# bioscan-ml/bioscan-clip

Hardware: AMD Instinct MI355X
Metric: paired samples/sec/node (I+D+T, global batch) + step MFMA-roofline % at 1/2/4/8 GPU (higher is better)
Workload: dtype bf16; 1 GPU; configs[2]: Image+DNA+Text (LoRA ViT-B/16 + LoRA BarcodeBERT + BERT-small), local batch 256, 224x224 images + 133-token barcodes, local-batch InfoNCE, fused AdamW; local_batch=256, global_batch=256, parallelism=dp1, collectives=none (one process, local-batch loss)

## Files before the change

### bioscan-clip_amd/csrc/common.h

```cpp
#pragma once
#include <hip/hip_runtime.h>
#include <stdint.h>

#include "../../include/bsclip.h"

typedef unsigned short bf16_t;
typedef __attribute__((ext_vector_type(8))) __bf16 bf16x8;
typedef __attribute__((ext_vector_type(4))) float f32x4;
typedef __attribute__((ext_vector_type(16))) float f32x16;
typedef __attribute__((ext_vector_type(4))) unsigned short u16x4;
typedef __attribute__((ext_vector_type(8))) unsigned short u16x8;

#define BSCLIP_WAVE 64

void bsclip_set_error(const char* fmt, ...);
#define BSCLIP_REQUIRE(cond, ...)                    \
    do {                                             \
        if (!(cond)) {                               \
            bsclip_set_error(__VA_ARGS__);           \
            return BSCLIP_ERR_INVALID;               \
        }                                            \
    } while (0)
#define BSCLIP_LAUNCH_CHECK()                                                        \
    do {                                                                             \
// ... 217 lines not shown
}

static inline int ceil_div(int a, int b) { return (a + b - 1) / b; }

void bsclip_launch_slab_reduce_add(const float* partial, int nblocks, int n, float* out0, float* out1, int split, hipStream_t s);

void bsclip_launch_attn_fwd_x3(const float* qkv, int ld_qkv, int B, int S, int heads, const float* key_bias, float scale, float* ctx,
                               int ld_ctx, float* lse, const DropCfg& drop, bf16_t* ctx3, int ld_c3, hipStream_t s);
void bsclip_launch_attn_bwd_x3(const float* qkv, int ld_qkv, const float* dctx, int ld_dctx, const float* ctx, int ld_ctx, const float* lse,
                               int B, int S, int heads, const float* key_bias, float scale, float* dqkv, int ld_dqkv, const DropCfg& drop,
                               bf16_t* dqkv3, int ld_d3, hipStream_t s);

int bsclip_gemm_infonce(int mode, const void* A, int lda, const void* B, int ldb, void* C, int ldc, int M, int N, int K,
                        const int64_t* labels, const float* cnt, const float* lse_row, const float* lse_col, float* part,
                        float logit_scale, float coef, int n_valid, int row_base, void* stream);
```

### bioscan-clip_amd/csrc/gemm.hip

```cpp
#include <type_traits>

#include "common.h"

namespace {

constexpr int BK = 64;
constexpr int ROW_BYTES = BK * 2;

__device__ __forceinline__ int xcd_remap(int orig, int nwg) {
    const int q = nwg >> 3, r = nwg & 7, xcd = orig & 7;
    return (xcd < r ? xcd * (q + 1) : r * (q + 1) + (xcd - r) * q) + (orig >> 3);
}

struct EpiArgs {
    const float* bias;
    const float* resid;
    int ld_resid;
    unsigned char* aux;
    int ld_aux;
    DropCfg drop;
    int n_total;
    unsigned long long* diag;
    int pers_gw;
    const float* alpha;
// ... 131 lines not shown
        v += bf4_to_f32<F16>(r);
        *reinterpret_cast<uint2*>(static_cast<bf16_t*>(C) + (size_t)m * ldc + n) = f32_to_bf4<F16>(v);
    } else if constexpr (EPI == BSCLIP_EPI_PATCH_BF16) {
        const int b = m / 196, p = m - b * 196;
        const f32x4 pos = *reinterpret_cast<const f32x4*>(e.resid + (size_t)(1 + p) * e.ld_resid + n);
        v += pos;
        *reinterpret_cast<uint2*>(static_cast<bf16_t*>(C) + (size_t)(b * 197 + 1 + p) * ldc + n) = f32_to_bf4<F16>(v);
    }
}

template <int BM, int BN, int WAVES_M, int WAVES_N, int EPI, bool HAS_BIAS, bool F16 = false>
__global__ __launch_bounds__(WAVES_M* WAVES_N * 64) void gemm_nt_kernel(const bf16_t* __restrict__ A, int lda,
                                                                         const bf16_t* __restrict__ B, int ldb,
                                                                         void* __restrict__ C, int ldc, int M, int N,
                                                                         int K, int tiles_n, EpiArgs e) {
    constexpr int NW = WAVES_M * WAVES_N;
    constexpr int WTM = BM / WAVES_M, WTN = BN / WAVES_N;
    if constexpr (epi_is_resid(EPI)) BSCLIP_DROP_RESOLVE(e.drop);
    constexpr int TM = WTM / 16, TN = WTN / 16;
    constexpr int A_BYTES = BM * ROW_BYTES, B_BYTES = BN * ROW_BYTES;
    constexpr int STAGE_BYTES = A_BYTES + B_BYTES;
    constexpr int A_PER_WAVE = BM / 8 / NW, B_PER_WAVE = BN / 8 / NW;
    static_assert(BM % (8 * NW) == 0 && BN % (8 * NW) == 0, "staging split");
    __shared__ __attribute__((aligned(16))) char smem[2 * STAGE_BYTES];

    const int wg = xcd_remap(blockIdx.x, gridDim.x);
    const int tile_n = wg % tiles_n, tile_m = wg / tiles_n;
    const int m0 = tile_m * BM, n0 = tile_n * BN;

    const int tid = threadIdx.x, lane = tid & 63;
    const int wave = __builtin_amdgcn_readfirstlane(tid >> 6);
    const int wm = wave / WAVES_N, wn = wave % WAVES_N;

    const bf16_t* a_src[A_PER_WAVE];
    const bf16_t* b_src[B_PER_WAVE];
#pragma unroll
    for (int i = 0; i < A_PER_WAVE; ++i) {
        const int row = (wave + i * NW) * 8 + (lane >> 3);
        const int c = (lane & 7) ^ ((row >> 1) & 7);
        const int grow = min(m0 + row, M - 1);
        a_src[i] = A + (size_t)grow * lda + c * 8;
    }
#pragma unroll
    for (int i = 0; i < B_PER_WAVE; ++i) {
        const int row = (wave + i * NW) * 8 + (lane >> 3);
        const int c = (lane & 7) ^ ((row >> 1) & 7);
        const int grow = min(n0 + row, N - 1);
        b_src[i] = B + (size_t)grow * ldb + c * 8;
    }
    auto stage = [&](int buf, int k0) {
        char* sA = smem + buf * STAGE_BYTES;
        char* sB = sA + A_BYTES;
#pragma unroll
        for (int i = 0; i < A_PER_WAVE; ++i) glds16(a_src[i] + k0, sA + (wave + i * NW) * 1024);
#pragma unroll
        for (int i = 0; i < B_PER_WAVE; ++i) glds16(b_src[i] + k0, sB + (wave + i * NW) * 1024);
    };

    const int fr = lane & 15, fq = lane >> 4;
    const int sw = fr >> 1;
    const int a_off0 = (wm * WTM + fr) * ROW_BYTES + ((fq ^ sw) << 4);
    const int b_off0 = (wn * WTN + fr) * ROW_BYTES + ((fq ^ sw) << 4);

    f32x4 acc[TM][TN];
#pragma unroll
    for (int i = 0; i < TM; ++i)
#pragma unroll
        for (int j = 0; j < TN; ++j) acc[i][j] = f32x4{0.f, 0.f, 0.f, 0.f};

    const int nk = K / BK;
    stage(0, 0);
    __syncthreads();

    for (int t = 0; t < nk; ++t) {
        const int cur = t & 1;
        if (t + 1 < nk) stage(cur ^ 1, (t + 1) * BK);
        const char* sA = smem + cur * STAGE_BYTES;
        const char* sB = sA + A_BYTES;
#pragma unroll
        for (int ks = 0; ks < 2; ++ks) {
            bf16x8 af[TM], bfr[TN];
#pragma unroll
            for (int j = 0; j < TN; ++j)
                bfr[j] = *reinterpret_cast<const bf16x8*>(sB + ((b_off0 ^ (ks << 6)) + j * 16 * ROW_BYTES));
#pragma unroll
            for (int i = 0; i < TM; ++i)
                af[i] = *reinterpret_cast<const bf16x8*>(sA + ((a_off0 ^ (ks << 6)) + i * 16 * ROW_BYTES));
#pragma unroll
            for (int i = 0; i < TM; ++i)
#pragma unroll
                for (int j = 0; j < TN; ++j)
                    acc[i][j] = mfma16x16x32<F16>(bfr[j], af[i], acc[i][j]);
        }
        __syncthreads();
    }

    f32x4 bias[TN];
#pragma unroll
    for (int j = 0; j < TN; ++j) {
        bias[j] = f32x4{0.f, 0.f, 0.f, 0.f};
        if constexpr (HAS_BIAS) bias[j] = *reinterpret_cast<const f32x4*>(e.bias + n0 + wn * WTN + j * 16 + fq * 4);
    }
    if constexpr (HAS_BIAS) {
#pragma unroll
        for (int i = 0; i < TM; ++i)
#pragma unroll
            for (int j = 0; j < TN; ++j) acc[i][j] += bias[j];
    }
    auto store_rows = [&](auto guard) {
#pragma unroll
        for (int i = 0; i < TM; ++i) {
            const int m = m0 + wm * WTM + i * 16 + fr;
            if (!decltype(guard)::value || m < M) {
#pragma unroll
                for (int j = 0; j < TN; ++j) {
                    const int n = n0 + wn * WTN + j * 16 + fq * 4;
                    epilogue_store<EPI, F16>(acc[i][j], m, n, C, ldc, e);
                }
            }
        }
    };
    if (m0 + BM <= M) store_rows(std::false_type{});
    else store_rows(std::true_type{});
}

template <int EPI, bool HAS_BIAS, bool DIAG = false, int ABL = 0, int SCHED = 0, int OP = 0>
__global__ __launch_bounds__(512) void gemm_nt_pp_kernel(const bf16_t* __restrict__ A, int lda,
                                                          const bf16_t* __restrict__ B, int ldb, void* __restrict__ C,
                                                          int ldc, int M, int N, int K, int tiles_n, EpiArgs e) {
    static_assert(OP == 0 || (SCHED == 0 && ABL == 0), "fp8 / fp16 operands: production schedule only");
    constexpr bool FP8 = OP == 1 || OP == 2, F16 = OP == 3;
    if constexpr (EPI == BSCLIP_EPI_F32 && !HAS_BIAS && OP == 0) {
        A += (size_t)blockIdx.y * K;
        B += (size_t)blockIdx.y * K;
        C = static_cast<float*>(C) + (size_t)blockIdx.y * e.split_stride;
    }
    if constexpr (epi_is_resid(EPI)) BSCLIP_DROP_RESOLVE(e.drop);
    constexpr int ESZ = FP8 ? 1 : 2;
// ... 702 lines not shown
    const int tiles_m = ceil_div(M, BM), tiles_n = N / BN;
    hipLaunchKernelGGL((gemm_nt_kernel<BM, BN, WM, WN, EPI, HB, F16>), dim3(tiles_m * tiles_n), dim3(WM * WN * 64), 0, s, A,
                       lda, B, ldb, C, ldc, M, N, K, tiles_n, e);
}

bool g_lut_ready = false;

template <int EPI, bool HB, bool F16, int SCHED = 0>
void launch_pp(const bf16_t* A, int lda, const bf16_t* B, int ldb, void* C, int ldc, int M, int N, int K,
               const EpiArgs& e, hipStream_t s) {
    const int tiles_m = ceil_div(M, 256), tiles_n = N / 256;
    hipLaunchKernelGGL((gemm_nt_pp_kernel<EPI, HB, false, 0, F16 ? 0 : SCHED, F16 ? 3 : 0>), dim3(tiles_m * tiles_n), dim3(512), 0, s, A, lda, B,
                       ldb, C, ldc, M, N, K, tiles_n, e);
}

template <int EPI, bool HB, bool F16>
void launch_epi(const bf16_t* A, int lda, const bf16_t* B, int ldb, void* C, int ldc, int M, int N, int K,
                const EpiArgs& e, hipStream_t s) {
    if (EPI == BSCLIP_EPI_GELU_BF16 && !g_lut_ready) {
        hipLaunchKernelGGL(gelu_lut_init_kernel, dim3(ceil_div(GELU_LUT_N + 1, 256)), dim3(256), 0, s);
        g_lut_ready = true;
    }
    int tile = g_tile_override;
    if (tile == 0) {
        const long t256 = (long)ceil_div(M, 256) * (N / 256);
        if (N % 256 == 0 && t256 >= 192) tile = 4;
        else tile = 1;
        if (tile == 4 && N == 768 && K == 768 && t256 >= 500 && EPI != BSCLIP_EPI_GELU_BF16 && !g_duo_off) tile = 5;
        if (tile == 4 && pers_supported(EPI) && K <= g_pers_max_k && K >= 2 * BK && t256 >= g_pers_min_tiles && !g_pers_off) tile = 8;
    }
    if (F16 && tile == 5) tile = 4;
    if ((tile == 3 || tile == 4 || tile == 6 || tile == 7 || tile == 8) && N % 256 != 0) tile = 2;
    switch (tile) {
        case 4: launch_pp<EPI, HB, F16>(A, lda, B, ldb, C, ldc, M, N, K, e, s); break;
        case 5:
            if constexpr (!F16) launch_duo<EPI, HB>(A, lda, B, ldb, C, ldc, M, N, K, e, s);
            break;
        case 8:
            if constexpr (pers_supported(EPI)) {
                if (K >= 2 * BK && (size_t)M * lda * 2 < (1ull << 32) && (size_t)N * ldb * 2 < (1ull << 32)) {
                    launch_pers<EPI, HB, F16>(A, lda, B, ldb, C, ldc, M, N, K, e, s);
                    break;
                }
            }
            launch_pp<EPI, HB, F16>(A, lda, B, ldb, C, ldc, M, N, K, e, s);
            break;
#ifdef BSCLIP_DIAG
// ... 304 lines not shown
    e.n_total = N;
    e.drop = make_drop(0.f, 0);
    const int tiles_m = ceil_div(M, 256), tiles_n = N / 256;
    hipStream_t s = static_cast<hipStream_t>(stream);
    const bf16_t* a = static_cast<const bf16_t*>(A);
    const bf16_t* b = static_cast<const bf16_t*>(B);
    if (mode == 0) {
        BSCLIP_REQUIRE(part, "bsclip_gemm_infonce: part is null");
        hipLaunchKernelGGL((gemm_nt_pp_kernel<EPI_LSE_PART, false>), dim3(tiles_m * tiles_n), dim3(512), 0, s, a, lda, b, ldb, C,
                           ldc, M, N, K, tiles_n, e);
    } else {
        BSCLIP_REQUIRE(C && cnt && lse_row && lse_col && ldc % 3 == 0, "bsclip_gemm_infonce: pass 2 operands");
        hipLaunchKernelGGL((gemm_nt_pp_kernel<EPI_LOSS_W, false>), dim3(tiles_m * tiles_n), dim3(512), 0, s, a, lda, b, ldb, C,
                           ldc, M, N, K, tiles_n, e);
    }
    BSCLIP_LAUNCH_CHECK();
    return BSCLIP_OK;
}

extern "C" int bsclip_gemm_fp8(const void* A8, int lda, const void* B8, int ldb, void* C, int ldc, int M, int N, int K,
                               int epilogue, const bsclip_epi_args* args, const bsclip_fp8_args* f8, void* stream) {
    BSCLIP_REQUIRE(A8 && B8 && C && args && f8, "bsclip_gemm_fp8: null pointer");
    BSCLIP_REQUIRE(args->struct_size == sizeof(bsclip_epi_args) && f8->struct_size == sizeof(bsclip_fp8_args),
                   "bsclip_gemm_fp8: struct_size mismatch (epi %u/%zu, fp8 %u/%zu)", args->struct_size,
                   sizeof(bsclip_epi_args), f8->struct_size, sizeof(bsclip_fp8_args));
    BSCLIP_REQUIRE(M > 0 && N > 0 && K > 0 && K % 128 == 0 && N % 256 == 0, "bsclip_gemm_fp8: M=%d N=%d K=%d (K %% 128, N %% 256)",
                   M, N, K);
    BSCLIP_REQUIRE(lda >= K && ldb >= K && lda % 16 == 0 && ldb % 16 == 0, "bsclip_gemm_fp8: lda=%d ldb=%d (K=%d)", lda, ldb, K);
    BSCLIP_REQUIRE(ldc >= N && ldc % 4 == 0 && (epilogue != BSCLIP_EPI_GELU_FP8 || ldc % 16 == 0), "bsclip_gemm_fp8: ldc=%d", ldc);
    BSCLIP_REQUIRE((((uintptr_t)A8 | (uintptr_t)B8 | (uintptr_t)C) & 15) == 0, "bsclip_gemm_fp8: 16-B alignment");
// ... 96 lines not shown
```

### bioscan-clip_amd/csrc/loss.hip

```cpp
#include <math.h>

#include "common.h"

namespace {

typedef __attribute__((ext_vector_type(4))) unsigned u32x4;

__device__ __forceinline__ void split_bf(float x, bf16_t& hi, bf16_t& lo) {
    hi = f2bf(x);
    lo = f2bf(x - bf2f(hi));
}

__global__ __launch_bounds__(256) void loss_prep_kernel(const float* __restrict__ z, int N, int Np, int D,
                                                         float* __restrict__ zn, float* __restrict__ inv,
                                                         bf16_t* __restrict__ PA, bf16_t* __restrict__ PB) {
    const int lane = threadIdx.x & 63;
    const int row = (blockIdx.x * 256 + threadIdx.x) >> 6;
    if (row >= Np) return;
    float scale = 0.f;
    if (row < N) {
        float ss = 0.f;
        for (int c = lane * 4; c < D; c += 256) {
            const f32x4 v = *reinterpret_cast<const f32x4*>(z + (size_t)row * D + c);
            ss += (v[0] * v[0] + v[1] * v[1]) + (v[2] * v[2] + v[3] * v[3]);
        }
        ss = wave_sum(ss);
        scale = 1.0f / fmaxf(sqrtf(ss), 1e-12f);
    }
    if (lane == 0) inv[row] = scale;
    for (int c = lane * 4; c < D; c += 256) {
// ... 3 lines not shown
        bf16_t h[4], l[4];
#pragma unroll
        for (int i = 0; i < 4; ++i) split_bf(v[i], h[i], l[i]);
        const uint2 hh = {(unsigned)h[0] | ((unsigned)h[1] << 16), (unsigned)h[2] | ((unsigned)h[3] << 16)};
        const uint2 ll = {(unsigned)l[0] | ((unsigned)l[1] << 16), (unsigned)l[2] | ((unsigned)l[3] << 16)};
        bf16_t* pa = PA + (size_t)row * 3 * D + c;
        bf16_t* pb = PB + (size_t)row * 3 * D + c;
        *reinterpret_cast<uint2*>(pa) = hh;
        *reinterpret_cast<uint2*>(pa + D) = hh;
        *reinterpret_cast<uint2*>(pa + 2 * D) = ll;
        *reinterpret_cast<uint2*>(pb) = hh;
        *reinterpret_cast<uint2*>(pb + D) = ll;
        *reinterpret_cast<uint2*>(pb + 2 * D) = hh;
    }
}

__global__ __launch_bounds__(256) void loss_transpose_split_kernel(const float* __restrict__ zn, int Np, int D,
                                                                    bf16_t* __restrict__ PBt) {
    __shared__ float tile[64][65];
    const int r0 = blockIdx.y * 64, c0 = blockIdx.x * 64;
    const int tx = threadIdx.x & 63, ty = threadIdx.x >> 6;
    for (int i = ty; i < 64; i += 4) tile[i][tx] = zn[(size_t)(r0 + i) * D + c0 + tx];
    __syncthreads();
    for (int i = ty; i < 64; i += 4) {
        const float v = tile[tx][i];
        bf16_t h, l;
        split_bf(v, h, l);
        bf16_t* dst = PBt + (size_t)(c0 + i) * 3 * Np + r0 + tx;
        dst[0] = h;
        dst[Np] = l;
        dst[2 * Np] = h;
    }
}

__global__ void loss_count_kernel(const int64_t* __restrict__ labels, int N, float* __restrict__ cnt) {
    const int i = blockIdx.x * blockDim.x + threadIdx.x;
    if (i >= N) return;
    const int64_t li = labels[i];
    int c = 0;
    for (int j = 0; j < N; ++j) c += (labels[j] == li);
    cnt[i] = (float)c;
}

__global__ __launch_bounds__(256) void loss_row_reduce_kernel(const float* __restrict__ G, int row0, int nrows, int N,
                                                               int Np, float s, const int64_t* __restrict__ labels,
                                                               const float* __restrict__ cnt, float* __restrict__ lse,
                                                               float* __restrict__ contrib) {
    const int lane = threadIdx.x & 63;
    const int r = (blockIdx.x * 256 + threadIdx.x) >> 6;
    if (r >= nrows) return;
    const int row = row0 + r;
    const float* g = G + (size_t)r * Np;
    const int64_t li = labels[row];
    float m = -INFINITY;
    for (int j = lane; j < N; j += 64) m = fmaxf(m, g[j]);
    m = wave_max(m) * s;
    float se = 0.f, dot = 0.f;
    for (int j = lane; j < N; j += 64) {
        const float x = g[j] * s;
        se += __expf(x - m);
        if (labels[j] == li) dot += x;
    }
    se = wave_sum(se);
    dot = wave_sum(dot);
    const float l = m + __logf(se);
    if (lane == 0) {
        lse[row] = l;
        contrib[row] = cnt[row] * l - dot;
    }
}

__global__ __launch_bounds__(256) void loss_w_kernel(const float* __restrict__ G, int N, int Np, int row0, int n_local,
                                                      float s, float coef, const int64_t* __restrict__ labels,
                                                      const float* __restrict__ cnt, const float* __restrict__ lse_ab,
                                                      const float* __restrict__ lse_ba, bf16_t* __restrict__ W) {
    const long total = (long)n_local * Np;
    for (long it = (long)blockIdx.x * 256 + threadIdx.x; it < total; it += (long)gridDim.x * 256) {
        const int il = (int)(it / Np), j = (int)(it % Np);
        float w = 0.f;
        if (j < N) {
            const int i = row0 + il;
            const float x = G[(size_t)il * Np + j] * s;
            const float t = (labels[i] == labels[j]) ? 2.0f : 0.0f;
            w = coef * (cnt[i] * __expf(x - lse_ab[i]) + cnt[j] * __expf(x - lse_ba[j]) - t);
        }
        bf16_t h, l;
        split_bf(w, h, l);
        bf16_t* dst = W + (size_t)il * 3 * Np + j;
        dst[0] = h;
        dst[Np] = h;
        dst[2 * Np] = l;
    }
}

__global__ __launch_bounds__(256) void loss_final_kernel(const float* __restrict__ contrib, int nmod, int Np, int N, float scale,
                                                          float* __restrict__ loss_out) {
    __shared__ float red[256];
    float s = 0.f;
    for (int slot = 0; slot < nmod * nmod; ++slot) {
        if (slot / nmod == slot % nmod) continue;
        for (int i = threadIdx.x; i < N; i += 256) s += contrib[(size_t)slot * Np + i];
    }
    red[threadIdx.x] = s;
    __syncthreads();
    for (int o = 128; o > 0; o >>= 1) {
        if (threadIdx.x < o) red[threadIdx.x] += red[threadIdx.x + o];
        __syncthreads();
// ... 9 lines not shown
    const f32x4* p = reinterpret_cast<const f32x4*>(part) + (size_t)i * tiles;
    float m = -INFINITY;
    for (int t = 0; t < tiles; ++t) m = fmaxf(m, p[t][0]);
    float s = 0.f, dot = 0.f;
    for (int t = 0; t < tiles; ++t) {
        const f32x4 v = p[t];
        s += v[0] == -INFINITY ? 0.f : v[1] * __expf(v[0] - m);
        dot += v[2];
    }
    const float l = m + __logf(s);
    lse[i] = l;
    contrib[i] = cnt[i] * l - dot;
}

int g_infonce_impl = 0;

inline int64_t align4(int64_t x) { return (x + 3) & ~(int64_t)3; }

constexpr int SLAB_ROWS = 1024;

struct Layout {
    int Np, slab;
    int64_t zn, inv, PA, PB, PBt, G, W, lse, contrib, cnt, dacc, part, total;
};

Layout make_layout(int N, int nmod, int D) {
    Layout L;
    L.Np = (N + 255) / 256 * 256;
    L.slab = L.Np < SLAB_ROWS ? L.Np : SLAB_ROWS;
    const int64_t Np = L.Np, SL = L.slab;
    int64_t o = 0;
    L.zn = o;      o += align4((int64_t)nmod * Np * D);
    L.inv = o;     o += align4((int64_t)nmod * Np);
    L.PA = o;      o += align4((int64_t)nmod * Np * 3 * D / 2);
    L.PB = o;      o += align4((int64_t)nmod * Np * 3 * D / 2);
    L.PBt = o;     o += align4((int64_t)nmod * D * 3 * Np / 2);
    L.G = o;       o += align4(SL * Np);
    L.W = o;       o += align4(SL * 3 * Np / 2);
    L.lse = o;     o += align4((int64_t)nmod * nmod * Np);
    L.contrib = o; o += align4((int64_t)nmod * nmod * Np);
    L.cnt = o;     o += align4(Np);
    L.dacc = o;    o += align4((int64_t)nmod * Np * D);
    L.part = o;    o += align4(Np * (Np / 256) * 4);
    L.total = o;
    return L;
}

}

extern "C" int64_t bsclip_infonce_workspace_floats(int N, int nmod) {
    if (N <= 0 || nmod < 2 || nmod > 3) return -1;
    return make_layout(N, nmod, 768).total;
}
// ... 14 lines not shown
    float* zn = ws + L.zn;
    float* inv = ws + L.inv;
    bf16_t* PA = reinterpret_cast<bf16_t*>(ws + L.PA);
    bf16_t* PB = reinterpret_cast<bf16_t*>(ws + L.PB);
    bf16_t* PBt = reinterpret_cast<bf16_t*>(ws + L.PBt);
    float* G = ws + L.G;
    bf16_t* W = reinterpret_cast<bf16_t*>(ws + L.W);
    float* lse = ws + L.lse;
    float* contrib = ws + L.contrib;
    float* cnt = ws + L.cnt;
    float* dacc = ws + L.dacc;
    float* part = ws + L.part;
    const bool fused = g_infonce_impl == 2 || (g_infonce_impl == 0 && Np >= 2048);
    const size_t opA = (size_t)Np * 3 * D;
    const size_t opT = (size_t)D * 3 * Np;

    for (int m = 0; m < nmod; ++m) {
        BSCLIP_REQUIRE(z[m], "bsclip_infonce_fwd_bwd: z[%d] is null", m);
        hipLaunchKernelGGL(loss_prep_kernel, dim3(ceil_div(Np, 4)), dim3(256), 0, s, z[m], N, Np, D,
                           zn + (size_t)m * Np * D, inv + (size_t)m * Np, PA + m * opA, PB + m * opA);
        if (dz && n_local > 0)
            hipLaunchKernelGGL(loss_transpose_split_kernel, dim3(D / 64, Np / 64), dim3(256), 0, s,
                               zn + (size_t)m * Np * D, Np, D, PBt + m * opT);
    }
    hipLaunchKernelGGL(loss_count_kernel, dim3(ceil_div(N, 256)), dim3(256), 0, s, labels, N, cnt);
    BSCLIP_LAUNCH_CHECK();

    const int ndir = nmod * (nmod - 1);
    for (int a = 0; a < nmod; ++a)
        for (int b = 0; b < nmod; ++b) {
            if (a == b) continue;
            const int slot = a * nmod + b;
            if (fused) {
                int rc = bsclip_gemm_infonce(0, PA + a * opA, 3 * D, PB + b * opA, 3 * D, nullptr, 0, N, Np, 3 * D, labels, cnt,
                                             nullptr, nullptr, part, scale, 0.f, N, 0, stream);
                if (rc) return rc;
                hipLaunchKernelGGL(infonce_combine_kernel, dim3(ceil_div(N, 256)), dim3(256), 0, s, part, N, Np / 256, cnt,
                                   lse + (size_t)slot * Np, contrib + (size_t)slot * Np);
                continue;
            }
            for (int r0 = 0; r0 < N; r0 += L.slab) {
                const int nr = N - r0 < L.slab ? N - r0 : L.slab;
                int rc = bsclip_gemm_bf16(PA + a * opA + (size_t)r0 * 3 * D, 3 * D, PB + b * opA, 3 * D, G, Np, nr, Np,
// ... 62 lines not shown
```

### bioscan-clip_amd/csrc/norm.hip

```cpp
#include "common.h"

namespace {

constexpr int LN_BLOCK = 256;

__device__ __forceinline__ float reduce8(float (&p)[8], int lane) {
    float q[4];
    const bool hi5 = lane & 32;
#pragma unroll
    for (int i = 0; i < 4; ++i) {
        const float send = hi5 ? p[i] : p[i + 4];
        const float keep = hi5 ? p[i + 4] : p[i];
        q[i] = keep + __shfl_xor(send, 32, 64);
    }
    float r2[2];
    const bool hi4 = lane & 16;
#pragma unroll
    for (int i = 0; i < 2; ++i) {
        const float send = hi4 ? q[i] : q[i + 2];
        const float keep = hi4 ? q[i + 2] : q[i];
        r2[i] = keep + __shfl_xor(send, 16, 64);
    }
    const bool hi3 = lane & 8;
    float v = (hi3 ? r2[1] : r2[0]) + __shfl_xor(hi3 ? r2[0] : r2[1], 8, 64);
// ... 279 lines not shown
    const float* xr = x + (size_t)row * D;
    float ss = 0.f;
    for (int c = lane * 4; c < D; c += 256) {
        const f32x4 v = *reinterpret_cast<const f32x4*>(xr + c);
        ss += (v[0] * v[0] + v[1] * v[1]) + (v[2] * v[2] + v[3] * v[3]);
    }
    ss = wave_sum(ss);
    const float inv = 1.0f / fmaxf(sqrtf(ss), 1e-12f);
    if (inv_norm && lane == 0) inv_norm[row] = inv;
    for (int c = lane * 4; c < D; c += 256) {
        const f32x4 v = *reinterpret_cast<const f32x4*>(xr + c);
        *reinterpret_cast<f32x4*>(y + (size_t)row * D + c) = v * inv;
    }
}

__global__ __launch_bounds__(LN_BLOCK) void l2norm_bwd_kernel(const float* __restrict__ y,
                                                               const float* __restrict__ inv_norm,
                                                               const float* __restrict__ dy, int M, int D,
                                                               float* __restrict__ dx) {
    const int lane = threadIdx.x & 63;
    const int row = (blockIdx.x * LN_BLOCK + threadIdx.x) >> 6;
    if (row >= M) return;
    const float* yr = y + (size_t)row * D;
    const float* gr = dy + (size_t)row * D;
    float dot = 0.f;
    for (int c = lane * 4; c < D; c += 256) {
        const f32x4 a = *reinterpret_cast<const f32x4*>(yr + c);
        const f32x4 g = *reinterpret_cast<const f32x4*>(gr + c);
        dot += (a[0] * g[0] + a[1] * g[1]) + (a[2] * g[2] + a[3] * g[3]);
    }
    dot = wave_sum(dot);
    const float inv = inv_norm[row];
    for (int c = lane * 4; c < D; c += 256) {
        const f32x4 a = *reinterpret_cast<const f32x4*>(yr + c);
        const f32x4 g = *reinterpret_cast<const f32x4*>(gr + c);
        *reinterpret_cast<f32x4*>(dx + (size_t)row * D + c) = (g - a * dot) * inv;
    }
}

int ln_grid(int M, int resident_per_cu = 8) {
    const int blocks = ceil_div(M, LN_BLOCK / 64);
    const int cap = 256 * resident_per_cu;
    return blocks < cap ? blocks : cap;
}

}

#define LN_FWD_LAUNCH(HH, XB, LO)                                                                              \
    hipLaunchKernelGGL((layernorm_fwd_kernel<HH, XB, LO>), dim3(ln_grid(M, LO ? 5 : 8)), dim3(LN_BLOCK), 0, s, x, ld_x, M, \
                       gamma, beta, eps, static_cast<bf16_t*>(y_bf16), ld_y, y_f32, lora_a, stats, drop,               \
                       static_cast<bf16_t*>(nullptr), 0, static_cast<bf16_t*>(y_split3), ld_y3)
#define LN_FWD16_LAUNCH(HH, XB, LO)                                                                            \
// ... 124 lines not shown
    BSCLIP_REQUIRE(x && y && M > 0 && D % 4 == 0, "bsclip_l2norm_fwd: bad args (M=%d D=%d)", M, D);
    hipLaunchKernelGGL(l2norm_fwd_kernel, dim3(ceil_div(M, LN_BLOCK / 64)), dim3(LN_BLOCK), 0,
                       static_cast<hipStream_t>(stream), x, M, D, y, inv_norm);
    BSCLIP_LAUNCH_CHECK();
    return BSCLIP_OK;
}

extern "C" int bsclip_l2norm_bwd(const float* y, const float* inv_norm, const float* dy, int M, int D, float* dx,
                                 void* stream) {
    BSCLIP_REQUIRE(y && inv_norm && dy && dx && M > 0 && D % 4 == 0, "bsclip_l2norm_bwd: bad args (M=%d D=%d)", M, D);
    hipLaunchKernelGGL(l2norm_bwd_kernel, dim3(ceil_div(M, LN_BLOCK / 64)), dim3(LN_BLOCK), 0,
                       static_cast<hipStream_t>(stream), y, inv_norm, dy, M, D, dx);
    BSCLIP_LAUNCH_CHECK();
    return BSCLIP_OK;
}
```

Baseline: 6494 paired samples/s.

## Batch InfoNCE loss kernels across modality pairs into grouped launches

Adds a batched path for the small-batch InfoNCE loss. It runs the prep, transpose, the six pairwise logit GEMMs, the row reductions, the weight computation, the gradient GEMMs and the L2-norm backward as grid-z or grid-y batched launches instead of a per-pair loop. The aim is to cut kernel launch count and raise occupancy on small 256-row problems. In exchange it keeps the G and W buffers for all pairs in memory. The GEMM body moves into a shared include so the batched kernel can reuse it.

```diff
diff --git a/bioscan-clip_amd/csrc/common.h b/bioscan-clip_amd/csrc/common.h
--- a/bioscan-clip_amd/csrc/common.h
+++ b/bioscan-clip_amd/csrc/common.h
@@ -255,3 +255,21 @@
 int bsclip_gemm_infonce(int mode, const void* A, int lda, const void* B, int ldb, void* C, int ldc, int M, int N, int K,
                         const int64_t* labels, const float* cnt, const float* lse_row, const float* lse_col, float* part,
                         float logit_scale, float coef, int n_valid, int row_base, void* stream);
+
+constexpr int BSCLIP_GEMM_BATCH_MAX = 6;
+struct bsclip_gemm_batch {
+    const void* A[BSCLIP_GEMM_BATCH_MAX];
+    const void* B[BSCLIP_GEMM_BATCH_MAX];
+    void* C[BSCLIP_GEMM_BATCH_MAX];
+};
+bool bsclip_gemm_batched_ok(int M, int N, int K, int epilogue);
+int bsclip_gemm_bf16_batched(const bsclip_gemm_batch& t, int nb, int lda, int ldb, int ldc, int M, int N, int K, int epilogue,
+                             void* stream);
+
+struct bsclip_l2norm_bwd_batch {
+    const float* y[3];
+    const float* inv_norm[3];
+    const float* dy[3];
+    float* dx[3];
+};
+int bsclip_l2norm_bwd_batched(const bsclip_l2norm_bwd_batch& t, int nb, int M, int D, void* stream);
diff --git a/bioscan-clip_amd/csrc/gemm.hip b/bioscan-clip_amd/csrc/gemm.hip
--- a/bioscan-clip_amd/csrc/gemm.hip
+++ b/bioscan-clip_amd/csrc/gemm.hip
@@ -169,114 +169,21 @@
                                                                          const bf16_t* __restrict__ B, int ldb,
                                                                          void* __restrict__ C, int ldc, int M, int N,
                                                                          int K, int tiles_n, EpiArgs e) {
-    constexpr int NW = WAVES_M * WAVES_N;
-    constexpr int WTM = BM / WAVES_M, WTN = BN / WAVES_N;
-    if constexpr (epi_is_resid(EPI)) BSCLIP_DROP_RESOLVE(e.drop);
-    constexpr int TM = WTM / 16, TN = WTN / 16;
-    constexpr int A_BYTES = BM * ROW_BYTES, B_BYTES = BN * ROW_BYTES;
-    constexpr int STAGE_BYTES = A_BYTES + B_BYTES;
-    constexpr int A_PER_WAVE = BM / 8 / NW, B_PER_WAVE = BN / 8 / NW;
-    static_assert(BM % (8 * NW) == 0 && BN % (8 * NW) == 0, "staging split");
-    __shared__ __attribute__((aligned(16))) char smem[2 * STAGE_BYTES];
-
-    const int wg = xcd_remap(blockIdx.x, gridDim.x);
-    const int tile_n = wg % tiles_n, tile_m = wg / tiles_n;
-    const int m0 = tile_m * BM, n0 = tile_n * BN;
-
-    const int tid = threadIdx.x, lane = tid & 63;
-    const int wave = __builtin_amdgcn_readfirstlane(tid >> 6);
-    const int wm = wave / WAVES_N, wn = wave % WAVES_N;
-
-    const bf16_t* a_src[A_PER_WAVE];
-    const bf16_t* b_src[B_PER_WAVE];
-#pragma unroll
-    for (int i = 0; i < A_PER_WAVE; ++i) {
-        const int row = (wave + i * NW) * 8 + (lane >> 3);
-        const int c = (lane & 7) ^ ((row >> 1) & 7);
-        const int grow = min(m0 + row, M - 1);
-        a_src[i] = A + (size_t)grow * lda + c * 8;
-    }
-#pragma unroll
-    for (int i = 0; i < B_PER_WAVE; ++i) {
-        const int row = (wave + i * NW) * 8 + (lane >> 3);
-        const int c = (lane & 7) ^ ((row >> 1) & 7);
-        const int grow = min(n0 + row, N - 1);
-        b_src[i] = B + (size_t)grow * ldb + c * 8;
-    }
-    auto stage = [&](int buf, int k0) {
-        char* sA = smem + buf * STAGE_BYTES;
-        char* sB = sA + A_BYTES;
-#pragma unroll
-        for (int i = 0; i < A_PER_WAVE; ++i) glds16(a_src[i] + k0, sA + (wave + i * NW) * 1024);
-#pragma unroll
-        for (int i = 0; i < B_PER_WAVE; ++i) glds16(b_src[i] + k0, sB + (wave + i * NW) * 1024);
-    };
-
-    const int fr = lane & 15, fq = lane >> 4;
-    const int sw = fr >> 1;
-    const int a_off0 = (wm * WTM + fr) * ROW_BYTES + ((fq ^ sw) << 4);
-    const int b_off0 = (wn * WTN + fr) * ROW_BYTES + ((fq ^ sw) << 4);
-
-    f32x4 acc[TM][TN];
-#pragma unroll
-    for (int i = 0; i < TM; ++i)
-#pragma unroll
-        for (int j = 0; j < TN; ++j) acc[i][j] = f32x4{0.f, 0.f, 0.f, 0.f};
-
-    const int nk = K / BK;
-    stage(0, 0);
-    __syncthreads();
-
-    for (int t = 0; t < nk; ++t) {
-        const int cur = t & 1;
-        if (t + 1 < nk) stage(cur ^ 1, (t + 1) * BK);
-        const char* sA = smem + cur * STAGE_BYTES;
-        const char* sB = sA + A_BYTES;
-#pragma unroll
-        for (int ks = 0; ks < 2; ++ks) {
-            bf16x8 af[TM], bfr[TN];
-#pragma unroll
-            for (int j = 0; j < TN; ++j)
-                bfr[j] = *reinterpret_cast<const bf16x8*>(sB + ((b_off0 ^ (ks << 6)) + j * 16 * ROW_BYTES));
-#pragma unroll
-            for (int i = 0; i < TM; ++i)
-                af[i] = *reinterpret_cast<const bf16x8*>(sA + ((a_off0 ^ (ks << 6)) + i * 16 * ROW_BYTES));
-#pragma unroll
-            for (int i = 0; i < TM; ++i)
-#pragma unroll
-                for (int j = 0; j < TN; ++j)
-                    acc[i][j] = mfma16x16x32<F16>(bfr[j], af[i], acc[i][j]);
-        }
-        __syncthreads();
-    }
-
-    f32x4 bias[TN];
-#pragma unroll
-    for (int j = 0; j < TN; ++j) {
-        bias[j] = f32x4{0.f, 0.f, 0.f, 0.f};
-        if constexpr (HAS_BIAS) bias[j] = *reinterpret_cast<const f32x4*>(e.bias + n0 + wn * WTN + j * 16 + fq * 4);
-    }
-    if constexpr (HAS_BIAS) {
-#pragma unroll
-        for (int i = 0; i < TM; ++i)
-#pragma unroll
-            for (int j = 0; j < TN; ++j) acc[i][j] += bias[j];
-    }
-    auto store_rows = [&](auto guard) {
-#pragma unroll
-        for (int i = 0; i < TM; ++i) {
-            const int m = m0 + wm * WTM + i * 16 + fr;
-            if (!decltype(guard)::value || m < M) {
-#pragma unroll
-                for (int j = 0; j < TN; ++j) {
-                    const int n = n0 + wn * WTN + j * 16 + fq * 4;
-                    epilogue_store<EPI, F16>(acc[i][j], m, n, C, ldc, e);
-                }
-            }
-        }
-    };
-    if (m0 + BM <= M) store_rows(std::false_type{});
-    else store_rows(std::true_type{});
+#include "gemm_nt_body.h"
+}
+
+template <int BM, int BN, int WAVES_M, int WAVES_N, int EPI>
+__global__ __launch_bounds__(WAVES_M* WAVES_N * 64) void gemm_nt_batched_kernel(bsclip_gemm_batch t, int lda, int ldb, int ldc,
+                                                                                 int M, int N, int K, int tiles_n, EpiArgs e) {
+    constexpr bool HAS_BIAS = false, F16 = false;
+    const bf16_t* __restrict__ A = static_cast<const bf16_t*>(t.A[blockIdx.z]);
+    const bf16_t* __restrict__ B = static_cast<const bf16_t*>(t.B[blockIdx.z]);
+    void* __restrict__ C = t.C[blockIdx.z];
+    if constexpr (epi_is_resid(EPI)) {
+        e.resid = static_cast<const float*>(C);
+        e.ld_resid = ldc;
+    }
+#include "gemm_nt_body.h"
 }
 
 template <int EPI, bool HAS_BIAS, bool DIAG = false, int ABL = 0, int SCHED = 0, int OP = 0>
@@ -1009,13 +916,8 @@
                        ldb, C, ldc, M, N, K, tiles_n, e);
 }
 
-template <int EPI, bool HB, bool F16>
-void launch_epi(const bf16_t* A, int lda, const bf16_t* B, int ldb, void* C, int ldc, int M, int N, int K,
-                const EpiArgs& e, hipStream_t s) {
-    if (EPI == BSCLIP_EPI_GELU_BF16 && !g_lut_ready) {
-        hipLaunchKernelGGL(gelu_lut_init_kernel, dim3(ceil_div(GELU_LUT_N + 1, 256)), dim3(256), 0, s);
-        g_lut_ready = true;
-    }
+template <int EPI, bool F16>
+int pick_tile(int M, int N, int K) {
     int tile = g_tile_override;
     if (tile == 0) {
         const long t256 = (long)ceil_div(M, 256) * (N / 256);
@@ -1026,6 +928,17 @@
     }
     if (F16 && tile == 5) tile = 4;
     if ((tile == 3 || tile == 4 || tile == 6 || tile == 7 || tile == 8) && N % 256 != 0) tile = 2;
+    return tile;
+}
+
+template <int EPI, bool HB, bool F16>
+void launch_epi(const bf16_t* A, int lda, const bf16_t* B, int ldb, void* C, int ldc, int M, int N, int K,
+                const EpiArgs& e, hipStream_t s) {
+    if (EPI == BSCLIP_EPI_GELU_BF16 && !g_lut_ready) {
+        hipLaunchKernelGGL(gelu_lut_init_kernel, dim3(ceil_div(GELU_LUT_N + 1, 256)), dim3(256), 0, s);
+        g_lut_ready = true;
+    }
+    const int tile = pick_tile<EPI, F16>(M, N, K);
     switch (tile) {
         case 4: launch_pp<EPI, HB, F16>(A, lda, B, ldb, C, ldc, M, N, K, e, s); break;
         case 5:
@@ -1360,6 +1273,39 @@
         hipLaunchKernelGGL((gemm_nt_pp_kernel<EPI_LOSS_W, false>), dim3(tiles_m * tiles_n), dim3(512), 0, s, a, lda, b, ldb, C,
                            ldc, M, N, K, tiles_n, e);
     }
+    BSCLIP_LAUNCH_CHECK();
+    return BSCLIP_OK;
+}
+
+bool bsclip_gemm_batched_ok(int M, int N, int K, int epilogue) {
+    if (M <= 0 || N <= 0 || N % 128 != 0 || K <= 0 || K % 64 != 0) return false;
+    if (epilogue == BSCLIP_EPI_F32) return pick_tile<BSCLIP_EPI_F32, false>(M, N, K) == 1;
+    if (epilogue == BSCLIP_EPI_RESID_F32) return pick_tile<BSCLIP_EPI_RESID_F32, false>(M, N, K) == 1;
+    return false;
+}
+
+int bsclip_gemm_bf16_batched(const bsclip_gemm_batch& t, int nb, int lda, int ldb, int ldc, int M, int N, int K, int epilogue,
+                             void* stream) {
+    BSCLIP_REQUIRE(nb >= 1 && nb <= BSCLIP_GEMM_BATCH_MAX, "bsclip_gemm_bf16_batched: nb=%d", nb);
+    BSCLIP_REQUIRE(bsclip_gemm_batched_ok(M, N, K, epilogue), "bsclip_gemm_bf16_batched: M=%d N=%d K=%d epilogue=%d is not a 128x128 shape",
+                   M, N, K, epilogue);
+    BSCLIP_REQUIRE(lda >= K && ldb >= K && lda % 8 == 0 && ldb % 8 == 0 && ldc >= N && ldc % 4 == 0,
+                   "bsclip_gemm_bf16_batched: lda=%d ldb=%d ldc=%d", lda, ldb, ldc);
+    for (int i = 0; i < nb; ++i)
+        BSCLIP_REQUIRE(t.A[i] && t.B[i] && t.C[i] && (((uintptr_t)t.A[i] | (uintptr_t)t.B[i] | (uintptr_t)t.C[i]) & 15) == 0,
+                       "bsclip_gemm_bf16_batched: operand %d null or not 16-B aligned", i);
+    EpiArgs e{};
+    e.n_total = N;
+    e.drop = make_drop(0.f, 0);
+    const int tiles_m = ceil_div(M, 128), tiles_n = N / 128;
+    const dim3 grid(tiles_m * tiles_n, 1, nb);
+    hipStream_t s = static_cast<hipStream_t>(stream);
+    if (epilogue == BSCLIP_EPI_F32)
+        hipLaunchKernelGGL((gemm_nt_batched_kernel<128, 128, 2, 2, BSCLIP_EPI_F32>), grid, dim3(256), 0, s, t, lda, ldb, ldc, M, N, K,
+                           tiles_n, e);
+    else
+        hipLaunchKernelGGL((gemm_nt_batched_kernel<128, 128, 2, 2, BSCLIP_EPI_RESID_F32>), grid, dim3(256), 0, s, t, lda, ldb, ldc, M,
+                           N, K, tiles_n, e);
     BSCLIP_LAUNCH_CHECK();
     return BSCLIP_OK;
 }
diff --git a/bioscan-clip_amd/csrc/gemm_nt_body.h b/bioscan-clip_amd/csrc/gemm_nt_body.h
--- /dev/null
+++ b/bioscan-clip_amd/csrc/gemm_nt_body.h
@@ -0,0 +1,108 @@
+    constexpr int NW = WAVES_M * WAVES_N;
+    constexpr int WTM = BM / WAVES_M, WTN = BN / WAVES_N;
+    if constexpr (epi_is_resid(EPI)) BSCLIP_DROP_RESOLVE(e.drop);
+    constexpr int TM = WTM / 16, TN = WTN / 16;
+    constexpr int A_BYTES = BM * ROW_BYTES, B_BYTES = BN * ROW_BYTES;
+    constexpr int STAGE_BYTES = A_BYTES + B_BYTES;
+    constexpr int A_PER_WAVE = BM / 8 / NW, B_PER_WAVE = BN / 8 / NW;
+    static_assert(BM % (8 * NW) == 0 && BN % (8 * NW) == 0, "staging split");
+    __shared__ __attribute__((aligned(16))) char smem[2 * STAGE_BYTES];
+
+    const int wg = xcd_remap(blockIdx.x, gridDim.x);
+    const int tile_n = wg % tiles_n, tile_m = wg / tiles_n;
+    const int m0 = tile_m * BM, n0 = tile_n * BN;
+
+    const int tid = threadIdx.x, lane = tid & 63;
+    const int wave = __builtin_amdgcn_readfirstlane(tid >> 6);
+    const int wm = wave / WAVES_N, wn = wave % WAVES_N;
+
+    const bf16_t* a_src[A_PER_WAVE];
+    const bf16_t* b_src[B_PER_WAVE];
+#pragma unroll
+    for (int i = 0; i < A_PER_WAVE; ++i) {
+        const int row = (wave + i * NW) * 8 + (lane >> 3);
+        const int c = (lane & 7) ^ ((row >> 1) & 7);
+        const int grow = min(m0 + row, M - 1);
+        a_src[i] = A + (size_t)grow * lda + c * 8;
+    }
+#pragma unroll
+    for (int i = 0; i < B_PER_WAVE; ++i) {
+        const int row = (wave + i * NW) * 8 + (lane >> 3);
+        const int c = (lane & 7) ^ ((row >> 1) & 7);
+        const int grow = min(n0 + row, N - 1);
+        b_src[i] = B + (size_t)grow * ldb + c * 8;
+    }
+    auto stage = [&](int buf, int k0) {
+        char* sA = smem + buf * STAGE_BYTES;
+        char* sB = sA + A_BYTES;
+#pragma unroll
+        for (int i = 0; i < A_PER_WAVE; ++i) glds16(a_src[i] + k0, sA + (wave + i * NW) * 1024);
+#pragma unroll
+        for (int i = 0; i < B_PER_WAVE; ++i) glds16(b_src[i] + k0, sB + (wave + i * NW) * 1024);
+    };
+
+    const int fr = lane & 15, fq = lane >> 4;
+    const int sw = fr >> 1;
+    const int a_off0 = (wm * WTM + fr) * ROW_BYTES + ((fq ^ sw) << 4);
+    const int b_off0 = (wn * WTN + fr) * ROW_BYTES + ((fq ^ sw) << 4);
+
+    f32x4 acc[TM][TN];
+#pragma unroll
+    for (int i = 0; i < TM; ++i)
+#pragma unroll
+        for (int j = 0; j < TN; ++j) acc[i][j] = f32x4{0.f, 0.f, 0.f, 0.f};
+
+    const int nk = K / BK;
+    stage(0, 0);
+    __syncthreads();
+
+    for (int t = 0; t < nk; ++t) {
+        const int cur = t & 1;
+        if (t + 1 < nk) stage(cur ^ 1, (t + 1) * BK);
+        const char* sA = smem + cur * STAGE_BYTES;
+        const char* sB = sA + A_BYTES;
+#pragma unroll
+        for (int ks = 0; ks < 2; ++ks) {
+            bf16x8 af[TM], bfr[TN];
+#pragma unroll
+            for (int j = 0; j < TN; ++j)
+                bfr[j] = *reinterpret_cast<const bf16x8*>(sB + ((b_off0 ^ (ks << 6)) + j * 16 * ROW_BYTES));
+#pragma unroll
+            for (int i = 0; i < TM; ++i)
+                af[i] = *reinterpret_cast<const bf16x8*>(sA + ((a_off0 ^ (ks << 6)) + i * 16 * ROW_BYTES));
+#pragma unroll
+            for (int i = 0; i < TM; ++i)
+#pragma unroll
+                for (int j = 0; j < TN; ++j)
+                    acc[i][j] = mfma16x16x32<F16>(bfr[j], af[i], acc[i][j]);
+        }
+        __syncthreads();
+    }
+
+    f32x4 bias[TN];
+#pragma unroll
+    for (int j = 0; j < TN; ++j) {
+        bias[j] = f32x4{0.f, 0.f, 0.f, 0.f};
+        if constexpr (HAS_BIAS) bias[j] = *reinterpret_cast<const f32x4*>(e.bias + n0 + wn * WTN + j * 16 + fq * 4);
+    }
+    if constexpr (HAS_BIAS) {
+#pragma unroll
+        for (int i = 0; i < TM; ++i)
+#pragma unroll
+            for (int j = 0; j < TN; ++j) acc[i][j] += bias[j];
+    }
+    auto store_rows = [&](auto guard) {
+#pragma unroll
+        for (int i = 0; i < TM; ++i) {
+            const int m = m0 + wm * WTM + i * 16 + fr;
+            if (!decltype(guard)::value || m < M) {
+#pragma unroll
+                for (int j = 0; j < TN; ++j) {
+                    const int n = n0 + wn * WTN + j * 16 + fq * 4;
+                    epilogue_store<EPI, F16>(acc[i][j], m, n, C, ldc, e);
+                }
+            }
+        }
+    };
+    if (m0 + BM <= M) store_rows(std::false_type{});
+    else store_rows(std::true_type{});
diff --git a/bioscan-clip_amd/csrc/loss.hip b/bioscan-clip_amd/csrc/loss.hip
--- a/bioscan-clip_amd/csrc/loss.hip
+++ b/bioscan-clip_amd/csrc/loss.hip
@@ -1,4 +1,5 @@
 #include <math.h>
+#include <stdlib.h>
 
 #include "common.h"
 
@@ -11,9 +12,17 @@
     lo = f2bf(x - bf2f(hi));
 }
 
-__global__ __launch_bounds__(256) void loss_prep_kernel(const float* __restrict__ z, int N, int Np, int D,
-                                                         float* __restrict__ zn, float* __restrict__ inv,
-                                                         bf16_t* __restrict__ PA, bf16_t* __restrict__ PB) {
+struct ModPtrs {
+    const float* z[3];
+};
+__device__ __host__ __forceinline__ void pair_ab(int p, int nmod, int& a, int& b) {
+    a = p / (nmod - 1);
+    b = p % (nmod - 1);
+    b += (b >= a);
+}
+
+__device__ __forceinline__ void loss_prep_rows(const float* __restrict__ z, int N, int Np, int D, float* __restrict__ zn,
+                                               float* __restrict__ inv, bf16_t* __restrict__ PA, bf16_t* __restrict__ PB) {
     const int lane = threadIdx.x & 63;
     const int row = (blockIdx.x * 256 + threadIdx.x) >> 6;
     if (row >= Np) return;
@@ -47,9 +56,19 @@
         *reinterpret_cast<uint2*>(pb + 2 * D) = hh;
     }
 }
-
-__global__ __launch_bounds__(256) void loss_transpose_split_kernel(const float* __restrict__ zn, int Np, int D,
-                                                                    bf16_t* __restrict__ PBt) {
+__global__ __launch_bounds__(256) void loss_prep_kernel(const float* __restrict__ z, int N, int Np, int D,
+                                                         float* __restrict__ zn, float* __restrict__ inv,
+                                                         bf16_t* __restrict__ PA, bf16_t* __restrict__ PB) {
+    loss_prep_rows(z, N, Np, D, zn, inv, PA, PB);
+}
+__global__ __launch_bounds__(256) void loss_prep_batched_kernel(ModPtrs src, int N, int Np, int D, float* __restrict__ zn,
+                                                                 float* __restrict__ inv, bf16_t* __restrict__ PA,
+                                                                 bf16_t* __restrict__ PB) {
+    const size_t m = blockIdx.y;
+    loss_prep_rows(src.z[m], N, Np, D, zn + m * Np * D, inv + m * Np, PA + m * Np * 3 * D, PB + m * Np * 3 * D);
+}
+
+__device__ __forceinline__ void loss_transpose_split_tile(const float* __restrict__ zn, int Np, int D, bf16_t* __restrict__ PBt) {
     __shared__ float tile[64][65];
     const int r0 = blockIdx.y * 64, c0 = blockIdx.x * 64;
     const int tx = threadIdx.x & 63, ty = threadIdx.x >> 6;
@@ -65,6 +84,15 @@
         dst[2 * Np] = h;
     }
 }
+__global__ __launch_bounds__(256) void loss_transpose_split_kernel(const float* __restrict__ zn, int Np, int D,
+                                                                    bf16_t* __restrict__ PBt) {
+    loss_transpose_split_tile(zn, Np, D, PBt);
+}
+__global__ __launch_bounds__(256) void loss_transpose_split_batched_kernel(const float* __restrict__ zn, int Np, int D,
+                                                                            bf16_t* __restrict__ PBt) {
+    const size_t m = blockIdx.z;
+    loss_transpose_split_tile(zn + m * Np * D, Np, D, PBt + m * D * 3 * Np);
+}
 
 __global__ void loss_count_kernel(const int64_t* __restrict__ labels, int N, float* __restrict__ cnt) {
     const int i = blockIdx.x * blockDim.x + threadIdx.x;
@@ -75,10 +103,9 @@
     cnt[i] = (float)c;
 }
 
-__global__ __launch_bounds__(256) void loss_row_reduce_kernel(const float* __restrict__ G, int row0, int nrows, int N,
-                                                               int Np, float s, const int64_t* __restrict__ labels,
-                                                               const float* __restrict__ cnt, float* __restrict__ lse,
-                                                               float* __restrict__ contrib) {
+__device__ __forceinline__ void loss_row_reduce_rows(const float* __restrict__ G, int row0, int nrows, int N, int Np, float s,
+                                                     const int64_t* __restrict__ labels, const float* __restrict__ cnt,
+                                                     float* __restrict__ lse, float* __restrict__ contrib) {
     const int lane = threadIdx.x & 63;
     const int r = (blockIdx.x * 256 + threadIdx.x) >> 6;
     if (r >= nrows) return;
@@ -102,11 +129,27 @@
         contrib[row] = cnt[row] * l - dot;
     }
 }
-
-__global__ __launch_bounds__(256) void loss_w_kernel(const float* __restrict__ G, int N, int Np, int row0, int n_local,
-                                                      float s, float coef, const int64_t* __restrict__ labels,
-                                                      const float* __restrict__ cnt, const float* __restrict__ lse_ab,
-                                                      const float* __restrict__ lse_ba, bf16_t* __restrict__ W) {
+__global__ __launch_bounds__(256) void loss_row_reduce_kernel(const float* __restrict__ G, int row0, int nrows, int N,
+                                                               int Np, float s, const int64_t* __restrict__ labels,
+                                                               const float* __restrict__ cnt, float* __restrict__ lse,
+                                                               float* __restrict__ contrib) {
+    loss_row_reduce_rows(G, row0, nrows, N, Np, s, labels, cnt, lse, contrib);
+}
+__global__ __launch_bounds__(256) void loss_row_reduce_batched_kernel(const float* __restrict__ G, int nmod, int N, int Np, float s,
+                                                                       const int64_t* __restrict__ labels,
+                                                                       const float* __restrict__ cnt, float* __restrict__ lse,
+                                                                       float* __restrict__ contrib) {
+    const int p = blockIdx.y;
+    int a, b;
+    pair_ab(p, nmod, a, b);
+    const size_t slot = a * nmod + b;
+    loss_row_reduce_rows(G + (size_t)p * Np * Np, 0, N, N, Np, s, labels, cnt, lse + slot * Np, contrib + slot * Np);
+}
+
+__device__ __forceinline__ void loss_w_elems(const float* __restrict__ G, int N, int Np, int row0, int n_local, float s,
+                                             float coef, const int64_t* __restrict__ labels, const float* __restrict__ cnt,
+                                             const float* __restrict__ lse_ab, const float* __restrict__ lse_ba,
+                                             bf16_t* __restrict__ W) {
     const long total = (long)n_local * Np;
     for (long it = (long)blockIdx.x * 256 + threadIdx.x; it < total; it += (long)gridDim.x * 256) {
         const int il = (int)(it / Np), j = (int)(it % Np);
@@ -124,6 +167,23 @@
         dst[Np] = h;
         dst[2 * Np] = l;
     }
+}
+__global__ __launch_bounds__(256) void loss_w_kernel(const float* __restrict__ G, int N, int Np, int row0, int n_local,
+                                                      float s, float coef, const int64_t* __restrict__ labels,
+                                                      const float* __restrict__ cnt, const float* __restrict__ lse_ab,
+                                                      const float* __restrict__ lse_ba, bf16_t* __restrict__ W) {
+    loss_w_elems(G, N, Np, row0, n_local, s, coef, labels, cnt, lse_ab, lse_ba, W);
+}
+__global__ __launch_bounds__(256) void loss_w_batched_kernel(const float* __restrict__ G, int nmod, int N, int Np, int row0,
+                                                              int n_local, float s, float coef,
+                                                              const int64_t* __restrict__ labels, const float* __restrict__ cnt,
+                                                              const float* __restrict__ lse, bf16_t* __restrict__ W,
+                                                              size_t w_stride) {
+    const int p = blockIdx.y;
+    int a, b;
+    pair_ab(p, nmod, a, b);
+    loss_w_elems(G + ((size_t)p * Np + row0) * Np, N, Np, row0, n_local, s, coef, labels, cnt, lse + (size_t)(a * nmod + b) * Np,
+                 lse + (size_t)(b * nmod + a) * Np, W + p * w_stride);
 }
 
 __global__ __launch_bounds__(256) void loss_final_kernel(const float* __restrict__ contrib, int nmod, int Np, int N, float scale,
@@ -163,6 +223,7 @@
 }
 
 int g_infonce_impl = 0;
+const bool g_infonce_batched_off = getenv("BSCLIP_INFONCE_BATCHED") && atoi(getenv("BSCLIP_INFONCE_BATCHED")) == 0;
 
 inline int64_t align4(int64_t x) { return (x + 3) & ~(int64_t)3; }
 
@@ -184,8 +245,9 @@
     L.PA = o;      o += align4((int64_t)nmod * Np * 3 * D / 2);
     L.PB = o;      o += align4((int64_t)nmod * Np * 3 * D / 2);
     L.PBt = o;     o += align4((int64_t)nmod * D * 3 * Np / 2);
-    L.G = o;       o += align4(SL * Np);
-    L.W = o;       o += align4(SL * 3 * Np / 2);
+    const int64_t keep = Np <= SLAB_ROWS ? nmod * (nmod - 1) : 1;
+    L.G = o;       o += align4(keep * SL * Np);
+    L.W = o;       o += align4(keep * SL * 3 * Np / 2);
     L.lse = o;     o += align4((int64_t)nmod * nmod * Np);
     L.contrib = o; o += align4((int64_t)nmod * nmod * Np);
     L.cnt = o;     o += align4(Np);
@@ -230,6 +292,75 @@
     const bool fused = g_infonce_impl == 2 || (g_infonce_impl == 0 && Np >= 2048);
     const size_t opA = (size_t)Np * 3 * D;
     const size_t opT = (size_t)D * 3 * Np;
+    const int ndir = nmod * (nmod - 1);
+    const bool want_dz = dz && n_local > 0;
+    const bool batched = g_infonce_impl == 0 && !g_infonce_batched_off && Np <= SLAB_ROWS &&
+                         bsclip_gemm_batched_ok(N, Np, 3 * D, BSCLIP_EPI_F32) &&
+                         (!want_dz || (bsclip_gemm_batched_ok(n_local, D, 3 * Np, BSCLIP_EPI_F32) &&
+                                       bsclip_gemm_batched_ok(n_local, D, 3 * Np, BSCLIP_EPI_RESID_F32)));
+    if (batched) {
+        ModPtrs src{};
+        for (int m = 0; m < nmod; ++m) {
+            BSCLIP_REQUIRE(z[m], "bsclip_infonce_fwd_bwd: z[%d] is null", m);
+            src.z[m] = z[m];
+        }
+        hipLaunchKernelGGL(loss_prep_batched_kernel, dim3(ceil_div(Np, 4), nmod), dim3(256), 0, s, src, N, Np, D, zn, inv, PA, PB);
+        if (want_dz)
+            hipLaunchKernelGGL(loss_transpose_split_batched_kernel, dim3(D / 64, Np / 64, nmod), dim3(256), 0, s, zn, Np, D, PBt);
+        hipLaunchKernelGGL(loss_count_kernel, dim3(ceil_div(N, 256)), dim3(256), 0, s, labels, N, cnt);
+        BSCLIP_LAUNCH_CHECK();
+
+        const size_t g_stride = (size_t)Np * Np;
+        const size_t w_stride = (size_t)L.slab * 3 * Np;
+        bsclip_gemm_batch gl{};
+        for (int p = 0; p < ndir; ++p) {
+            int a, b;
+            pair_ab(p, nmod, a, b);
+            gl.A[p] = PA + a * opA;
+            gl.B[p] = PB + b * opA;
+            gl.C[p] = G + p * g_stride;
+        }
+        int rc = bsclip_gemm_bf16_batched(gl, ndir, 3 * D, 3 * D, Np, N, Np, 3 * D, BSCLIP_EPI_F32, stream);
+        if (rc) return rc;
+        hipLaunchKernelGGL(loss_row_reduce_batched_kernel, dim3(ceil_div(N, 4), ndir), dim3(256), 0, s, G, nmod, N, Np, scale, labels,
+                           cnt, lse, contrib);
+        hipLaunchKernelGGL(loss_final_kernel, dim3(1), dim3(256), 0, s, contrib, nmod, Np, N, 1.0f / ((float)ndir * (float)N),
+                           loss_out);
+        BSCLIP_LAUNCH_CHECK();
+        if (!want_dz) return BSCLIP_OK;
+
+        const float coef = scale / ((float)ndir * (float)N);
+        for (int a = 0; a < nmod; ++a) BSCLIP_REQUIRE(dz[a], "bsclip_infonce_fwd_bwd: dz[%d] is null", a);
+        long blocks = ((long)n_local * Np + 255) / 256;
+        if (blocks > 4096) blocks = 4096;
+        hipLaunchKernelGGL(loss_w_batched_kernel, dim3((unsigned)blocks, ndir), dim3(256), 0, s, G, nmod, N, Np, row0, n_local, scale,
+                           coef, labels, cnt, lse, W, w_stride);
+        for (int k = 0; k < nmod - 1; ++k) {
+            bsclip_gemm_batch gd{};
+            for (int a = 0; a < nmod; ++a) {
+                const int p = a * (nmod - 1) + k;
+                int pa, b;
+                pair_ab(p, nmod, pa, b);
+                gd.A[a] = W + p * w_stride;
+                gd.B[a] = PBt + b * opT;
+                gd.C[a] = dacc + (size_t)a * Np * D;
+            }
+            rc = bsclip_gemm_bf16_batched(gd, nmod, 3 * Np, 3 * Np, D, n_local, D, 3 * Np,
+                                          k == 0 ? BSCLIP_EPI_F32 : BSCLIP_EPI_RESID_F32, stream);
+            if (rc) return rc;
+        }
+        bsclip_l2norm_bwd_batch nb{};
+        for (int a = 0; a < nmod; ++a) {
+            nb.y[a] = zn + ((size_t)a * Np + row0) * D;
+            nb.inv_norm[a] = inv + (size_t)a * Np + row0;
+            nb.dy[a] = dacc + (size_t)a * Np * D;
+            nb.dx[a] = dz[a];
+        }
+        rc = bsclip_l2norm_bwd_batched(nb, nmod, n_local, D, stream);
+        if (rc) return rc;
+        BSCLIP_LAUNCH_CHECK();
+        return BSCLIP_OK;
+    }
 
     for (int m = 0; m < nmod; ++m) {
         BSCLIP_REQUIRE(z[m], "bsclip_infonce_fwd_bwd: z[%d] is null", m);
@@ -242,7 +373,6 @@
     hipLaunchKernelGGL(loss_count_kernel, dim3(ceil_div(N, 256)), dim3(256), 0, s, labels, N, cnt);
     BSCLIP_LAUNCH_CHECK();
 
-    const int ndir = nmod * (nmod - 1);
     for (int a = 0; a < nmod; ++a)
         for (int b = 0; b < nmod; ++b) {
             if (a == b) continue;
diff --git a/bioscan-clip_amd/csrc/norm.hip b/bioscan-clip_amd/csrc/norm.hip
--- a/bioscan-clip_amd/csrc/norm.hip
+++ b/bioscan-clip_amd/csrc/norm.hip
@@ -317,10 +317,8 @@
     }
 }
 
-__global__ __launch_bounds__(LN_BLOCK) void l2norm_bwd_kernel(const float* __restrict__ y,
-                                                               const float* __restrict__ inv_norm,
-                                                               const float* __restrict__ dy, int M, int D,
-                                                               float* __restrict__ dx) {
+__device__ __forceinline__ void l2norm_bwd_rows(const float* __restrict__ y, const float* __restrict__ inv_norm,
+                                                const float* __restrict__ dy, int M, int D, float* __restrict__ dx) {
     const int lane = threadIdx.x & 63;
     const int row = (blockIdx.x * LN_BLOCK + threadIdx.x) >> 6;
     if (row >= M) return;
@@ -339,6 +337,18 @@
         const f32x4 g = *reinterpret_cast<const f32x4*>(gr + c);
         *reinterpret_cast<f32x4*>(dx + (size_t)row * D + c) = (g - a * dot) * inv;
     }
+}
+
+__global__ __launch_bounds__(LN_BLOCK) void l2norm_bwd_kernel(const float* __restrict__ y,
+                                                               const float* __restrict__ inv_norm,
+                                                               const float* __restrict__ dy, int M, int D,
+                                                               float* __restrict__ dx) {
+    l2norm_bwd_rows(y, inv_norm, dy, M, D, dx);
+}
+
+__global__ __launch_bounds__(LN_BLOCK) void l2norm_bwd_batched_kernel(bsclip_l2norm_bwd_batch t, int M, int D) {
+    const int p = blockIdx.y;
+    l2norm_bwd_rows(t.y[p], t.inv_norm[p], t.dy[p], M, D, t.dx[p]);
 }
 
 int ln_grid(int M, int resident_per_cu = 8) {
@@ -493,3 +503,13 @@
     BSCLIP_LAUNCH_CHECK();
     return BSCLIP_OK;
 }
+
+int bsclip_l2norm_bwd_batched(const bsclip_l2norm_bwd_batch& t, int nb, int M, int D, void* stream) {
+    BSCLIP_REQUIRE(nb >= 1 && nb <= 3 && M > 0 && D % 4 == 0, "bsclip_l2norm_bwd_batched: bad args (nb=%d M=%d D=%d)", nb, M, D);
+    for (int i = 0; i < nb; ++i)
+        BSCLIP_REQUIRE(t.y[i] && t.inv_norm[i] && t.dy[i] && t.dx[i], "bsclip_l2norm_bwd_batched: null pointer in problem %d", i);
+    hipLaunchKernelGGL(l2norm_bwd_batched_kernel, dim3(ceil_div(M, LN_BLOCK / 64), nb), dim3(LN_BLOCK), 0,
+                       static_cast<hipStream_t>(stream), t, M, D);
+    BSCLIP_LAUNCH_CHECK();
+    return BSCLIP_OK;
+}
```

Result: faster. 6607 paired samples/s (median of 6 runs) (+1.7%).
